# david-cortes/cmfrec

Measured on AMD Instinct MI355X. Metric: ALS rows/sec ((users+items)/iteration time), implicit ALS-CG k=50 fp64, higher is better.
Workload: dtype f64

## Files before the change

### cmfrec_amd/csrc/cg_kernels.hpp

```cpp
#pragma once
#include <hip/hip_runtime.h>
#include <stdint.h>
#include <type_traits>

#include "lanes.hpp"

namespace cmfhip {

constexpr int WAVE = 64;
constexpr int TILE = 64;
constexpr int MAX_W = 8;
#ifndef CMF_CG_WAVES_PER_SIMD
#define CMF_CG_WAVES_PER_SIMD 2
#endif
#ifndef CMF_CG_WAVES_PER_SIMD_F32
#define CMF_CG_WAVES_PER_SIMD_F32 3
#endif
#ifndef CMF_CG_WAVES_PER_SIMD_LOW
#define CMF_CG_WAVES_PER_SIMD_LOW 3
#endif
constexpr int CG_NTSEL_MAX_S = 7;
template <typename T, int W, int NRES_, int NTSEL = 0> constexpr int cg_waves_per_simd()
{
    if (sizeof(T) == 8 && NTSEL == 1 && W <= 8) return CMF_CG_WAVES_PER_SIMD_LOW;
    if (sizeof(T) == 4 && NTSEL == 1 && W <= 4 && NRES_ == 0) return CMF_CG_WAVES_PER_SIMD_F32 + 1;
    return (sizeof(T) == 4 && W <= 4 && NRES_ == 0) ? CMF_CG_WAVES_PER_SIMD_F32 : CMF_CG_WAVES_PER_SIMD;
}
constexpr int CG_NT_LOW = 6;
#ifndef CMF_CG_NT_F32
#define CMF_CG_NT_F32 1
#endif
#ifndef CMF_CG_NT_MIN_S
#define CMF_CG_NT_MIN_S 4
#endif

struct RowDesc {
    int row;
    int nnz;
    unsigned long long st;
};

constexpr int CG_NCOUNTERS = 64;
constexpr int CG_COUNTER_STRIDE = 32;

template <typename T>
__device__ __forceinline__ T cg_div(T num, T den)
{
#ifndef CMF_CG_IEEE_DIV
    if constexpr (sizeof(T) == 4) return num * __builtin_amdgcn_rcpf(den);
    else {
        double y = __builtin_amdgcn_rcp(den);
        double e = __builtin_fma(-den, y, 1.0);
        y = __builtin_fma(y, e, y);
        e = __builtin_fma(-den, y, 1.0);
        y = __builtin_fma(y, e, y);
        double q = num * y;
        const double r = __builtin_fma(-den, q, num);
        return __builtin_fma(r, y, q);
    }
#else
    return num / den;
#endif
}

template <typename V>
__device__ __forceinline__ V lds_g(const V *p) { return *p; }

template <typename T>
struct CgParams {
    T *A;
    size_t lda;
    const T *B;
    size_t ldb;
    int k;
    const size_t *indptr;
    const int *indices;
    const T *values;
    const T *bias_sub;
    const T *weights = nullptr;
    const T *wsum = nullptr;
    const int *order;
    const RowDesc *desc;
    int nrows;
    const T *BtB;
    T lam, lam_last;
    int scale_lam, scale_bias_const;
    int max_cg_steps;
    int precond;
    int koff = 0, kc = 0;
    const T *CtC = nullptr;
    const T *UC = nullptr;
    T w_side = 0;
    int rows_with_u = 0;
    int row_first = 0;
    const size_t *indptr2 = nullptr;
    const int *indices2 = nullptr;
    const T *values2 = nullptr;
    const T *C2 = nullptr;
    int *counter = nullptr;
    int p_side = 0, scale_lam_sideinfo = 0;
    const T *Bi = nullptr;
    const T *BiTBi = nullptr;
    int ki = 0;
    T w_imp = 0;
    const T *rconst = nullptr;
    size_t ldr = 0;
    int gx = 0;
#ifdef CMF_CG_DEBUG
    int dbg = 0;
#endif
#ifdef CMF_CG_TICKS
    unsigned long long *ticks = nullptr;
#endif
};
#ifdef CMF_CG_TICKS
#define CMF_TICK() __builtin_amdgcn_s_memtime()
__device__ __forceinline__ void cg_ticks_flush(unsigned long long *t, int slot, unsigned long long wait, unsigned long long pass, unsigned long long rows,
                                               unsigned long long total, int lane)
{
    if (t != nullptr && lane == 0) {
        atomicAdd(t + 4 * slot + 0, wait); atomicAdd(t + 4 * slot + 1, pass); atomicAdd(t + 4 * slot + 2, rows); atomicAdd(t + 4 * slot + 3, total);
    }
}
#endif
#ifdef CMF_CG_DEBUG
#define CMF_DBG(P, bit) (((P).dbg & (bit)) != 0)
#else
#define CMF_DBG(P, bit) false
#endif
template <int NT, int S, typename TILE, typename T>
__device__ __forceinline__ void dbg_fill_tile(TILE &tile, T val)
{
#pragma unroll
    for (int t = 0; t < NT; t++)
#pragma unroll
        for (int s = 0; s < S; s++) tile.set(t, s, val);
}

template <typename T>
__device__ __forceinline__ T wave_sum(T v) { return lanes::wave_sum(v); }

template <typename T, int NT, int I>
__device__ __forceinline__ T treduce8_low_first(const T (&v)[8], bool h)
{
    if constexpr (I + 4 < NT) {
        T keep = h ? v[I + 4] : v[I];
        return keep + lanes::recv_xor4(v[I], v[I + 4]);
    } else return v[I] + lanes::xor4_lower(v[I]);
}
template <typename T, int NT = 8>
__device__ __forceinline__ T treduce8_low(const T (&v)[8], int lane)
{
    static_assert(NT >= 4 && NT <= 8, "entries per lane group");
    T u[4], q[2];
    bool h = (lane & 4) != 0;
    u[0] = treduce8_low_first<T, NT, 0>(v, h); u[1] = treduce8_low_first<T, NT, 1>(v, h);
    u[2] = treduce8_low_first<T, NT, 2>(v, h); u[3] = treduce8_low_first<T, NT, 3>(v, h);
    h = (lane & 2) != 0;
#pragma unroll
    for (int i = 0; i < 2; i++) {
        T keep = h ? u[i + 2] : u[i];
        T send = h ? u[i] : u[i + 2];
        q[i] = keep + lanes::xor2(send);
    }
    h = (lane & 1) != 0;
    T keep = h ? q[1] : q[0];
    T send = h ? q[0] : q[1];
    return keep + lanes::xor1(send);
}

template <typename T>
__device__ __forceinline__ T treduce8_high(const T (&v)[8], int lane)
{
    T u[4], q[2];
#pragma unroll
    for (int i = 0; i < 4; i++) u[i] = lanes::tswap32_add(v[i], v[i + 4]);
#pragma unroll
    for (int i = 0; i < 2; i++) q[i] = lanes::tswap16_add(u[i], u[i + 2]);
    const bool h = (lane & 8) != 0;
    T keep = h ? q[1] : q[0];
    return keep + lanes::recv_xor8(q[0], q[1]);
}

#ifndef CMF_PASS_VECTOR_LDS
#define CMF_PASS_VECTOR_LDS 2
#endif
template <typename T> constexpr bool pass_vector_in_lds() { return CMF_PASS_VECTOR_LDS == 1 || (CMF_PASS_VECTOR_LDS == 2 && sizeof(T) == 8); }
template <typename T, int S>
__device__ __forceinline__ void replicate(T vdist, T (&vrep)[S], int lane);
template <typename T, int S, int GR = 8>
__device__ __forceinline__ void pass_vector_lds(T vdist, T (&vrep)[S], T (&wts)[8], int lane, T *__restrict__ pv)
{
    const int jj = lane >> 3, ll = lane & 7;
    pv[lane] = vdist;
    __builtin_amdgcn_wave_barrier();
#pragma unroll
    for (int s = 0; s < S; s++) vrep[s] = pv[ll + 8 * s];
    const T *wp = pv + GR * jj;
#pragma unroll
    for (int t = 0; t < GR; t++) wts[t] = wp[t];
    __builtin_amdgcn_wave_barrier();
}

__host__ __device__ constexpr int gram_ld(int S) { return 8 * S + 1; }
#ifndef CMF_GRAM_ROWS_BY_K
#define CMF_GRAM_ROWS_BY_K 1
#endif
template <typename T> __host__ __device__ constexpr int gram_rows(int S) { return (CMF_GRAM_ROWS_BY_K && pass_vector_in_lds<T>()) ? S : 8; }
__host__ __device__ constexpr int gram_ld_rows(int S, int GR)
{
    if (GR == 8) return gram_ld(S);
    int ld = 8 * S;
    while ((S * ld) % 32 != 8 && (S * ld) % 32 != 24) ld++;
    return ld;
}
__host__ __device__ constexpr int gram_ld2(int S) { return 8 * S + 2; }
template <typename T> __host__ __device__ constexpr int gram_elems(int S) { return sizeof(T) == 4 ? 64 * gram_ld2(S) : 64 * gram_ld(S); }
template <typename T, int S, int GR = 8> __device__ __forceinline__ int gram_index(int r, int c)
{
    if constexpr (sizeof(T) == 4) return 2 * ((r >> 1) * gram_ld2(S) + c) + (r & 1);
    else return r * gram_ld_rows(S, GR) + c;
}
template <typename T, int S, int GR = 8>
__device__ __forceinline__ void stage_gramian(T *__restrict__ G, const T *__restrict__ BtB, int k, int tid, int nthreads)
{
    static_assert(GR == 8 || sizeof(T) == 8, "rows by k: double precision");
    for (int e = tid; e < 8 * GR * 8 * S; e += nthreads) {
        const int r = e / (8 * S), c = e % (8 * S);
        G[gram_index<T, S, GR>(r, c)] = (r < k && c < k) ? BtB[(size_t)r * k + c] : T(0);
    }
}

template <typename T, int S>
struct RegTile {
    T v[8][S];
    __device__ __forceinline__ void set(int t, int s, T x) { v[t][s] = x; }
};
typedef float f32x2 __attribute__((ext_vector_type(2)));
template <int S>
struct RegTile<float, S> {
    f32x2 v[4][S];
    __device__ __forceinline__ void set(int t, int s, float x) { v[t >> 1][s][t & 1] = x; }
};

template <typename T>
struct PassAcc {
    T v[8];
    __device__ __forceinline__ void zero()
    {
#pragma unroll
        for (int s = 0; s < 8; s++) v[s] = T(0);
    }
    __device__ __forceinline__ void close(T (&out)[8]) const
    {
#pragma unroll
        for (int s = 0; s < 8; s++) out[s] = v[s];
    }
};
template <>
struct PassAcc<float> {
    f32x2 v[8];
    __device__ __forceinline__ void zero()
    {
#pragma unroll
        for (int s = 0; s < 8; s++) v[s] = f32x2{0.f, 0.f};
    }
    __device__ __forceinline__ void close(float (&out)[8]) const
    {
#pragma unroll
        for (int s = 0; s < 8; s++) out[s] = v[s][0] + v[s][1];
    }
};

#ifndef CMF_CG_EARLY_GATHER
#define CMF_CG_EARLY_GATHER 0
#endif
struct NoAfter {
    template <typename TAG> __device__ __forceinline__ void operator()(TAG) const {}
};
template <int S, typename ACC>
__device__ __forceinline__ void pin_acc(ACC &out)
{
#pragma unroll
    for (int s = 0; s < S; s++) asm volatile("" : "+v"(out.v[s]));
}
template <int TS, typename T, int S, typename TILE>
__device__ __forceinline__ void load_tile_slot(TILE &tile, const char *base, unsigned ldb_bytes, unsigned it, int col_last)
{
    const T *rp = reinterpret_cast<const T *>(base + (unsigned long long)it * ldb_bytes);
#pragma unroll
    for (int s = 0; s < S; s++) tile.set(TS, s, rp[(s < S - 1) ? 8 * s : col_last]);
}

template <typename T, int S, int NT = 8>
__device__ __forceinline__ void load_tile(RegTile<T, S> &tile, const T *__restrict__ Bm, size_t ldb,
                                          int k, int my_idx, int cnt, int lane)
{
    const int jj = lane >> 3, ll = lane & 7;
    int its[8];
    its[0] = lanes::bcast8<0>(my_idx); its[1] = lanes::bcast8<1>(my_idx); its[2] = lanes::bcast8<2>(my_idx);
    its[3] = lanes::bcast8<3>(my_idx);
    if (NT > 4) its[4] = lanes::bcast8<4>(my_idx);
    if (NT > 5) its[5] = lanes::bcast8<5>(my_idx);
    if (NT > 6) its[6] = lanes::bcast8<6>(my_idx);
    if (NT > 7) its[7] = lanes::bcast8<7>(my_idx);
    const int first_idx = __builtin_amdgcn_readfirstlane(my_idx);
    const int col_last = min(ll + 8 * (S - 1), k - 1) - ll;
    const char *base = reinterpret_cast<const char *>(Bm + ll);
    const unsigned ldb_bytes = (unsigned)(ldb * sizeof(T));
#pragma unroll
    for (int t = 0; t < NT; t++) {
        const unsigned it = (unsigned)(((jj * NT + t) < cnt) ? its[t] : first_idx);
        const T *rp = reinterpret_cast<const T *>(base + (unsigned long long)it * ldb_bytes);
#pragma unroll
        for (int s = 0; s < S; s++) tile.set(t, s, rp[(s < S - 1) ? 8 * s : col_last]);
    }
}

template <typename T, bool IMPLICIT, int MODE>
__device__ __forceinline__ T pass_weight(T coef, T x, bool valid, T g = T(1))
{
    T w;
    if (IMPLICIT) {
        if (MODE == 0) w = -(coef - T(1)) * x - coef;
        else           w = coef * (x - T(1)) + coef;
    } else {
        if (MODE == 0) w = -((coef - x) * g);
        else           w = coef * g;
    }
    return valid ? w : T(0);
}

template <typename T>
__device__ __forceinline__ T row_lam_mult(const CgParams<T> &P, int row, int nnz)
{
    return (P.wsum != nullptr) ? P.wsum[row] : (T)nnz;
}
template <typename T, bool IMPLICIT>
__device__ __forceinline__ T entry_weight(const CgParams<T> &P, size_t pos)
{
    if (IMPLICIT) return T(1);
    return (P.weights != nullptr) ? P.weights[pos] : T(1);
}

template <int S, bool IMPLICIT, int MODE, int NT = 8, bool INIT = false, typename AFTER = NoAfter>
__device__ __forceinline__ void tile_pass_f32(const RegTile<float, S> &tile, const float (&vrep)[S], float x, bool valid,
                                          PassAcc<float> &out, int lane, float g = 1.f, AFTER after = AFTER())
{
    static_assert(NT % 2 == 0, "single precision: the entries of a lane group travel in pairs");
    float c[8];
#pragma unroll
    for (int q = 0; q < NT / 2; q++) {
        f32x2 acc = f32x2{0.f, 0.f};
#pragma unroll
        for (int s = 0; s < S; s++) acc += tile.v[q][s] * f32x2{vrep[s], vrep[s]};
        c[2 * q] = acc[0]; c[2 * q + 1] = acc[1];
    }
    float coef = treduce8_low<float, NT>(c, lane);
    const float w = pass_weight<float, IMPLICIT, MODE>(coef, x, valid, g);
    float wts[8];
    wts[0] = lanes::bcast8<0>(w); wts[1] = lanes::bcast8<1>(w); wts[2] = lanes::bcast8<2>(w); wts[3] = lanes::bcast8<3>(w);
    if (NT > 4) { wts[4] = lanes::bcast8<4>(w); wts[5] = lanes::bcast8<5>(w); }
    if (NT > 6) { wts[6] = lanes::bcast8<6>(w); wts[7] = lanes::bcast8<7>(w); }
    if constexpr (std::is_same<AFTER, NoAfter>::value) {
#pragma unroll
    for (int q = 0; q < NT / 2; q++) {
        const f32x2 w2 = f32x2{wts[2 * q], wts[2 * q + 1]};
#pragma unroll
        for (int s = 0; s < S; s++) out.v[s] = (INIT && q == 0) ? w2 * tile.v[q][s] : out.v[s] + w2 * tile.v[q][s];
    }
    } else {
        static_for<0, NT / 2>([&](auto qc) {
            constexpr int q = decltype(qc)::value;
            const f32x2 w2 = f32x2{wts[2 * q], wts[2 * q + 1]};
#pragma unroll
            for (int s = 0; s < S; s++) out.v[s] = (INIT && q == 0) ? w2 * tile.v[q][s] : out.v[s] + w2 * tile.v[q][s];
            pin_acc<S>(out);
            after(std::integral_constant<int, 2 * q>{});
            after(std::integral_constant<int, 2 * q + 1>{});
        });
    }
    if constexpr (INIT) {
#pragma unroll
        for (int s = S; s < 8; s++) out.v[s] = f32x2{0.f, 0.f};
    }
}

template <typename T, int S, bool IMPLICIT, int MODE, int NT = 8, bool INIT = false, typename AFTER = NoAfter>
__device__ __forceinline__ void tile_pass(const RegTile<T, S> &tile, const T (&vrep)[S], T x, bool valid,
                                          PassAcc<T> &out, int lane, T g = T(1), AFTER after = AFTER())
{
    if constexpr (std::is_same<T, float>::value) {
        tile_pass_f32<S, IMPLICIT, MODE, NT, INIT, AFTER>(tile, vrep, x, valid, out, lane, g, after);
    } else {
    T c[8];
#pragma unroll
    for (int t = 0; t < NT; t++) {
        T acc = T(0);
#pragma unroll
        for (int s = 0; s < S; s++) acc += tile.v[t][s] * vrep[s];
        c[t] = acc;
    }
    T coef = treduce8_low<T, NT>(c, lane);
    const T w = pass_weight<T, IMPLICIT, MODE>(coef, x, valid, g);
    T wts[8];
    wts[0] = lanes::bcast8<0>(w); wts[1] = lanes::bcast8<1>(w); wts[2] = lanes::bcast8<2>(w); wts[3] = lanes::bcast8<3>(w);
    if (NT > 4) wts[4] = lanes::bcast8<4>(w);
    if (NT > 5) wts[5] = lanes::bcast8<5>(w);
    if (NT > 6) wts[6] = lanes::bcast8<6>(w);
    if (NT > 7) wts[7] = lanes::bcast8<7>(w);
    if constexpr (std::is_same<AFTER, NoAfter>::value) {
#pragma unroll
    for (int t = 0; t < NT; t++) {
#pragma unroll
        for (int s = 0; s < S; s++) out.v[s] = (INIT && t == 0) ? wts[t] * tile.v[t][s] : out.v[s] + wts[t] * tile.v[t][s];
    }
    } else {
        static_for<0, NT>([&](auto tc) {
            constexpr int t = decltype(tc)::value;
#pragma unroll
            for (int s = 0; s < S; s++) out.v[s] = (INIT && t == 0) ? wts[t] * tile.v[t][s] : out.v[s] + wts[t] * tile.v[t][s];
            pin_acc<S>(out);
            after(tc);
        });
    }
    if constexpr (INIT) {
#pragma unroll
        for (int s = S; s < 8; s++) out.v[s] = T(0);
    }
    }
}

template <typename T, int S, int W>
__device__ __forceinline__ void gram_pass(const T *__restrict__ G, T wdist, PassAcc<T> &out, int lane, int wr)
{
    constexpr int LD = gram_ld(S);
    const int jj = lane >> 3, ll = lane & 7;
    T wts[8];
    wts[0] = lanes::bcast8<0>(wdist); wts[1] = lanes::bcast8<1>(wdist); wts[2] = lanes::bcast8<2>(wdist);
    wts[3] = lanes::bcast8<3>(wdist); wts[4] = lanes::bcast8<4>(wdist); wts[5] = lanes::bcast8<5>(wdist);
    wts[6] = lanes::bcast8<6>(wdist); wts[7] = lanes::bcast8<7>(wdist);
    if constexpr (std::is_same<T, float>::value && W <= 4) {
#pragma unroll
        for (int q = 0; q < 4; q++) {
            if (W > 1 && (q % W) != wr) continue;
            const f32x2 *g = reinterpret_cast<const f32x2 *>(G) + (jj * 4 + q) * gram_ld2(S) + ll;
            const f32x2 w2 = f32x2{wts[2 * q], wts[2 * q + 1]};
#pragma unroll
            for (int s = 0; s < S; s++) out.v[s] += w2 * lds_g(g + 8 * s);
        }
    } else {
#pragma unroll
        for (int t = 0; t < 8; t++) {
            if (W > 1 && (t % W) != wr) continue;
#pragma unroll
            for (int s = 0; s < S; s++) {
                if constexpr (std::is_same<T, float>::value) out.v[s][0] += wts[t] * G[gram_index<T, S>(jj * 8 + t, ll + 8 * s)];
                else out.v[s] += wts[t] * lds_g(G + (jj * 8 + t) * LD + ll + 8 * s);
            }
        }
    }
}

template <bool NEG, typename T, int S, int W, int GR = 8>
__device__ __forceinline__ void gram_pass_w(const T *__restrict__ G, const T (&wts)[8], PassAcc<T> &out, int lane, int wr)
{
    constexpr int LD = gram_ld_rows(S, GR);
    const int jj = lane >> 3, ll = lane & 7;
    if constexpr (std::is_same<T, float>::value && W <= 4) {
#pragma unroll
        for (int q = 0; q < 4; q++) {
            if (W > 1 && (q % W) != wr) continue;
            const f32x2 *g = reinterpret_cast<const f32x2 *>(G) + (jj * 4 + q) * gram_ld2(S) + ll;
            const f32x2 w2 = f32x2{wts[2 * q], wts[2 * q + 1]};
#pragma unroll
            for (int s = 0; s < S; s++) out.v[s] = NEG ? out.v[s] - w2 * lds_g(g + 8 * s) : out.v[s] + w2 * lds_g(g + 8 * s);
        }
    } else {
#pragma unroll
        for (int t = 0; t < GR; t++) {
            if (W > 1 && (t % W) != wr) continue;
#pragma unroll
            for (int s = 0; s < S; s++) {
                if constexpr (std::is_same<T, float>::value) {
                    const float g = G[gram_index<T, S>(jj * 8 + t, ll + 8 * s)];
                    out.v[s][0] = NEG ? out.v[s][0] - wts[t] * g : out.v[s][0] + wts[t] * g;
                } else {
                    const T g = lds_g(G + (jj * GR + t) * LD + ll + 8 * s);
                    out.v[s] = NEG ? out.v[s] - wts[t] * g : out.v[s] + wts[t] * g;
                }
            }
        }
    }
}

template <typename T, int S>
__device__ __forceinline__ void replicate(T vdist, T (&vrep)[S], int lane)
{
    const int ll = lane & 7;
#pragma unroll
    for (int s = 0; s < S; s++) vrep[s] = __shfl(vdist, s * 8 + ll);
}

template <typename T, int S, bool IMPLICIT, int W, int RPB, bool GRAMX = false, int NRES_ = 0, int NTSEL = 0>
__global__ void __launch_bounds__(64 * W * RPB, (cg_waves_per_simd<T, W, NRES_, NTSEL>()))
cg_rows_kernel(const CgParams<T> P)
{
    constexpr bool GRAM = IMPLICIT || GRAMX;
    extern __shared__ __attribute__((aligned(16))) unsigned char smem_raw[];
    T *G = reinterpret_cast<T *>(smem_raw);
    T *red = G + (GRAM ? gram_elems<T>(S) : 0);
    const int tid = threadIdx.x;
    const int lane = tid & 63;
    const int wave = tid >> 6;
    const int grp = wave / W;
    const int wr = wave % W;
    const int k = P.k;

    const int nteams = gridDim.x * RPB;
    __shared__ int s_claim[4];
    constexpr bool PV = pass_vector_in_lds<T>();
    __shared__ __attribute__((aligned(16))) T s_pv[PV ? W * RPB : 1][PV ? 64 : 1];
    const int cslot = (blockIdx.x * RPB + grp) % CG_NCOUNTERS;
    int *const my_counter = P.counter + cslot * CG_COUNTER_STRIDE;
    const int cbase = nteams + cslot;
    auto issue_claim = [&]() -> int {
        int v = 0;
        if (wr == 0 && lane == 0) v = atomicAdd(my_counter, 1);
        return v;
    };
    int rnxt, rnn;
    if (W == 1) {
        const int c1 = issue_claim(), c2 = issue_claim();
        rnxt = cbase + CG_NCOUNTERS * __builtin_amdgcn_readfirstlane(c1);
        rnn = cbase + CG_NCOUNTERS * __builtin_amdgcn_readfirstlane(c2);
    } else if (wr == 0 && lane == 0) {
        s_claim[2] = cbase + CG_NCOUNTERS * atomicAdd(my_counter, 1);
        s_claim[3] = cbase + CG_NCOUNTERS * atomicAdd(my_counter, 1);
    }
    constexpr int GR = gram_rows<T>(S);
    if (GRAM) stage_gramian<T, S, GR>(G, P.BtB, k, tid, blockDim.x);
    if (GRAM || W > 1) __syncthreads();
    if (W > 1) { rnxt = s_claim[2]; rnn = s_claim[3]; }
    T *myred = red + (size_t)grp * 2 * W * 64;

    int buf = 0;
    static_assert(W == 1 || RPB == 1, "multi-wave teams own their workgroup (barriers are per row)");

    constexpr int NRES = NRES_ > 0 ? NRES_ : ((std::is_same<T, float>::value && W == 8) ? 2 : 1);
    static_assert(NRES == 1 || std::is_same<T, float>::value, "two resident tiles: single precision");
    static_assert(NTSEL == 0 || (S >= CMF_CG_NT_MIN_S && (sizeof(T) == 4 || S <= CG_NTSEL_MAX_S) && NRES_ == 0),
                  "launches by tile size: tiles by row length (double precision: k <= 56)");
    constexpr int NT_MIN = (S >= CMF_CG_NT_MIN_S && (CMF_CG_NT_F32 || !std::is_same<T, float>::value)) ? (std::is_same<T, float>::value ? 6 : 5) : 8;
    auto nt_of = [&](int nnz_) -> int {
        int nt = (nnz_ + 8 * W * NRES - 1) / (8 * W * NRES);
        if (std::is_same<T, float>::value) nt = (nt + 1) & ~1;
        return (nt > 8) ? 8 : (nt < NT_MIN ? NT_MIN : nt);
    };
    struct Pre { int idx; T x; T a; int idx2; T x2; T g; T g2; };
    auto load_desc = [&](int rix_) -> RowDesc {
        RowDesc d; d.row = 0; d.nnz = 0; d.st = 0;
        if (rix_ < P.nrows) d = P.desc[rix_];
        d.row = __builtin_amdgcn_readfirstlane(d.row);
        d.nnz = __builtin_amdgcn_readfirstlane(d.nnz);
        d.st = ((unsigned long long)(unsigned)__builtin_amdgcn_readfirstlane((int)(d.st >> 32)) << 32) |
               (unsigned)__builtin_amdgcn_readfirstlane((int)(d.st & 0xffffffffu));
        return d;
    };
    auto load_pre = [&](const RowDesc &d) -> Pre {
        Pre q; q.idx = 0; q.x = T(0); q.a = T(0); q.idx2 = 0; q.x2 = T(0); q.g = T(1); q.g2 = T(1);
        const int nt = nt_of(d.nnz), tl = 8 * nt;
        const int b = lane & 7;
        const int ent = (lane >> 3) * nt + b;
        const int cnt = min(tl, d.nnz - wr * tl);
        if (b < nt && ent < cnt) {
            const size_t pos = d.st + (size_t)wr * tl + ent;
            q.idx = P.indices[pos];
            q.x = P.values[pos];
            q.g = entry_weight<T, IMPLICIT>(P, pos);
            if (!IMPLICIT && P.bias_sub != nullptr) q.x -= P.bias_sub[q.idx];
        }
        if (NRES == 2) {
            const int cnt2 = min(tl, d.nnz - (wr + W) * tl);
            if (b < nt && ent < cnt2) {
                const size_t pos = d.st + (size_t)(wr + W) * tl + ent;
                q.idx2 = P.indices[pos];
                q.x2 = P.values[pos];
                q.g2 = entry_weight<T, IMPLICIT>(P, pos);
                if (!IMPLICIT && P.bias_sub != nullptr) q.x2 -= P.bias_sub[q.idx2];
            }
        }
        if (d.nnz > 0 && lane < k) q.a = P.A[(size_t)d.row * P.lda + lane];
        return q;
    };
    int rix = blockIdx.x * RPB + grp;
    RowDesc dcur = load_desc(rix);
    RowDesc dnxt = load_desc(rnxt);
    Pre pcur = load_pre(dcur);
    int pend = issue_claim();
    constexpr bool EARLY = CMF_CG_EARLY_GATHER != 0;
    constexpr int NT_MAX = (NTSEL == 1) ? CG_NT_LOW : 8;
    RegTile<T, S> tile_c;
    RegTile<T, (NRES == 2) ? S : 1> tile2_c;
    const char *const gbase = reinterpret_cast<const char *>(P.B + (lane & 7));
    const unsigned gldb = (unsigned)(P.ldb * sizeof(T));
    const int gcol_last = min((lane & 7) + 8 * (S - 1), k - 1) - (lane & 7);
    auto gather_slot = [&](auto &tl_, auto tc, int idx_, int first_idx_, int nt_, int cnt_) {
        constexpr int t = decltype(tc)::value;
        if constexpr (t < NT_MAX) {
            if (t < nt_) {
                const unsigned it_ = (unsigned)((((lane >> 3) * nt_ + t) < cnt_) ? lanes::bcast8<t>(idx_) : first_idx_);
                load_tile_slot<t, T, S>(tl_, gbase, gldb, it_, gcol_last);
            }
        }
    };
    struct Want { int nt0, cnt0, nt1, cnt1; };
    auto want_of = [&](const RowDesc &d) -> Want {
        Want w_;
        const int nt = nt_of(d.nnz), tl = 8 * nt;
        w_.cnt0 = min(tl, d.nnz - wr * tl);
        w_.nt0 = (w_.cnt0 > 0 && !CMF_DBG(P, 1)) ? nt : 0;
        w_.cnt1 = (NRES == 2) ? min(tl, d.nnz - (wr + W) * tl) : 0;
        w_.nt1 = (w_.cnt1 > 0 && !CMF_DBG(P, 1)) ? nt : 0;
        return w_;
    };
    auto gather_row = [&](const RowDesc &d, const Pre &q) {
        const Want w_ = want_of(d);
        const int f0 = __builtin_amdgcn_readfirstlane(q.idx);
        static_for<0, NT_MAX>([&](auto tc) { gather_slot(tile_c, tc, q.idx, f0, w_.nt0, w_.cnt0); });
        if constexpr (NRES == 2) {
            const int f1 = __builtin_amdgcn_readfirstlane(q.idx2);
            static_for<0, NT_MAX>([&](auto tc) { gather_slot(tile2_c, tc, q.idx2, f1, w_.nt1, w_.cnt1); });
        }
    };
    if constexpr (EARLY) gather_row(dcur, pcur);
#ifdef CMF_CG_TICKS
    unsigned long long tk_wait = 0, tk_pass = 0, tk_rows = 0;
    const unsigned long long tk_begin = CMF_TICK();
#endif
    int it = 0;
    RowDesc dnn;
    Pre pnxt;
    auto solve_row = [&](auto nt_tag) {
        constexpr int NT = decltype(nt_tag)::value;
        constexpr int TL = 8 * NT;
        const int row = dcur.row;
        const size_t st = dcur.st;
        const int nnz = dcur.nnz;
        const int ntiles = (nnz + TL - 1) / TL;
        const int my_ntiles = (ntiles > wr) ? (ntiles - wr + W - 1) / W : 0;
        const bool resident = NT < 8 || my_ntiles <= NRES;

        T lam = P.lam, lam_last = P.lam_last;
        if (GRAMX && P.kc > 0) {
            if (P.scale_lam || P.scale_lam_sideinfo) {
                T mult = row_lam_mult(P, row, nnz);
                if (P.scale_lam_sideinfo) mult += (T)P.p_side;
                lam *= mult; lam_last *= mult;
            }
        } else if (!IMPLICIT && P.scale_lam) {
            const T mult = row_lam_mult(P, row, nnz);
            lam *= mult;
            if (!P.scale_bias_const) lam_last *= mult;
        }
        T *arow = P.A + (size_t)row * P.lda;
        T a_d = pcur.a;

        RegTile<T, S> tile_r;
        RegTile<T, (NRES == 2) ? S : 1> tile2_r;
        auto &tile = [&]() -> RegTile<T, S> & { if constexpr (EARLY) return tile_c; else return tile_r; }();
        auto &tile2 = [&]() -> RegTile<T, (NRES == 2) ? S : 1> & { if constexpr (EARLY) return tile2_c; else return tile2_r; }();
        const int ent = (lane >> 3) * NT + (lane & 7);
        const bool lane_has = (NT == 8) || (lane & 7) < NT;
        const int cnt0 = min(TL, nnz - wr * TL);
        T x_res = pcur.x;
        const T g_res = pcur.g;
        bool valid_res = lane_has && ent < cnt0;
        if (CMF_DBG(P, 1)) dbg_fill_tile<8, S>(tile, (T)(pcur.idx & 3) * (T)0.001);
        else if (!EARLY && cnt0 > 0) load_tile<T, S, NT>(tile, P.B, P.ldb, k, pcur.idx, cnt0, lane);
        const int cnt1 = (NRES == 2) ? min(TL, nnz - (wr + W) * TL) : 0;
        const T x2_res = pcur.x2, g2_res = pcur.g2;
        const bool valid2_res = lane_has && ent < cnt1;
        if constexpr (NRES == 2) {
            if (!EARLY && cnt1 > 0 && !CMF_DBG(P, 1)) load_tile<T, S, NT>(tile2, P.B, P.ldb, k, pcur.idx2, cnt1, lane);
        }
        dnn = load_desc(rnn);
        pnxt = load_pre(dnxt);
#ifdef CMF_CG_TICKS
        const unsigned long long tk0 = CMF_TICK();
        asm volatile("s_waitcnt vmcnt(0)" ::: "memory");
        const unsigned long long tk1 = CMF_TICK();
        tk_wait += tk1 - tk0;
#endif

        auto run_pass = [&](T vdist, auto mode_tag, bool first, auto fin_tag) -> T {
            constexpr int MODE = decltype(mode_tag)::value;
            constexpr bool FIN = decltype(fin_tag)::value && EARLY;
            asm volatile("" ::: "memory");
            T vrep[S];
            T gw[8];
            if constexpr (PV) pass_vector_lds<T, S, GR>(vdist, vrep, gw, lane, &s_pv[wave][0]);
            else replicate<T, S>(vdist, vrep, lane);
            PassAcc<T> acc;
            acc.zero();
            if constexpr (FIN) {
                if (NT < 8 || NRES == 2 || resident) {
                    const Want nx = want_of(dnxt);
                    const int f0 = __builtin_amdgcn_readfirstlane(pnxt.idx);
                    auto after0 = [&](auto tc) { gather_slot(tile, tc, pnxt.idx, f0, nx.nt0, nx.cnt0); };
                    if (cnt0 > 0 && !CMF_DBG(P, 4)) {
                        tile_pass<T, S, IMPLICIT, MODE, NT>(tile, vrep, x_res, valid_res, acc, lane, g_res, after0);
                        static_for<NT, NT_MAX>(after0);
                    } else static_for<0, NT_MAX>(after0);
                    if constexpr (NRES == 2) {
                        const int f1 = __builtin_amdgcn_readfirstlane(pnxt.idx2);
                        auto after1 = [&](auto tc) { gather_slot(tile2, tc, pnxt.idx2, f1, nx.nt1, nx.cnt1); };
                        if (cnt1 > 0 && !CMF_DBG(P, 4)) {
                            tile_pass<T, S, IMPLICIT, MODE, NT>(tile2, vrep, x2_res, valid2_res, acc, lane, g2_res, after1);
                            static_for<NT, NT_MAX>(after1);
                        } else static_for<0, NT_MAX>(after1);
                    }
                } else {
                for (int tl = wr; tl < ntiles; tl += W) {
                    const int cnt = min(TL, nnz - tl * TL);
                    const bool valid = lane_has && ent < cnt;
                    const size_t pos = st + (size_t)tl * TL + ent;
                    int my_idx = valid ? P.indices[pos] : 0;
                    T x = valid ? P.values[pos] : T(0);
                    const T g = valid ? entry_weight<T, IMPLICIT>(P, pos) : T(1);
                    if (!IMPLICIT && P.bias_sub != nullptr && valid) x -= P.bias_sub[my_idx];
                    if (!CMF_DBG(P, 1)) load_tile<T, S, NT>(tile, P.B, P.ldb, k, my_idx, cnt, lane);
                    if (!CMF_DBG(P, 4)) tile_pass<T, S, IMPLICIT, MODE, NT>(tile, vrep, x, valid, acc, lane, g);
                }
                gather_row(dnxt, pnxt);
                }
            } else
            if constexpr (NRES == 2) {
                if (cnt0 > 0 && !CMF_DBG(P, 4)) tile_pass<T, S, IMPLICIT, MODE, NT>(tile, vrep, x_res, valid_res, acc, lane, g_res);
                if (cnt1 > 0 && !CMF_DBG(P, 4)) tile_pass<T, S, IMPLICIT, MODE, NT>(tile2, vrep, x2_res, valid2_res, acc, lane, g2_res);
            } else if constexpr (NT < 8) {
                if (cnt0 > 0 && !CMF_DBG(P, 4)) tile_pass<T, S, IMPLICIT, MODE, NT>(tile, vrep, x_res, valid_res, acc, lane, g_res);
            } else
            for (int tl = wr; tl < ntiles; tl += W) {
                T x, g; bool valid;
                const bool have = (tl == wr) && (resident || first);
                if (!have) {
                    const int cnt = min(TL, nnz - tl * TL);
                    valid = lane_has && ent < cnt;
                    const size_t pos = st + (size_t)tl * TL + ent;
                    int my_idx = valid ? P.indices[pos] : 0;
                    x = valid ? P.values[pos] : T(0);
                    g = valid ? entry_weight<T, IMPLICIT>(P, pos) : T(1);
                    if (!IMPLICIT && P.bias_sub != nullptr && valid) x -= P.bias_sub[my_idx];
                    if (!CMF_DBG(P, 1)) load_tile<T, S, NT>(tile, P.B, P.ldb, k, my_idx, cnt, lane);
                } else {
                    x = x_res; g = g_res; valid = valid_res;
                }
                if (!CMF_DBG(P, 4)) tile_pass<T, S, IMPLICIT, MODE, NT>(tile, vrep, x, valid, acc, lane, g);
            }
            if (GRAM && !CMF_DBG(P, 2)) {
                if constexpr (PV) gram_pass_w<MODE == 0, T, S, W, GR>(G, gw, acc, lane, wr);
                else gram_pass<T, S, W>(G, (MODE == 0) ? -vdist : vdist, acc, lane, wr);
            }
            T out[8];
            acc.close(out);
            T tot = treduce8_high<T>(out, lane);
            if (W > 1) {
                T *rb = myred + (size_t)buf * W * 64;
                rb[wr * 64 + lane] = tot;
                if (first && wr == 0 && lane == 0) s_claim[it & 1] = cbase + CG_NCOUNTERS * pend;
                __syncthreads();
                tot = T(0);
#pragma unroll
                for (int w = 0; w < W; w++) tot += rb[w * 64 + lane];
                buf ^= 1;
            }
            return tot;
        };

        T r_d = run_pass(a_d, std::integral_constant<int, 0>{}, true, std::false_type{});
        r_d -= lam * a_d;
        if (!IMPLICIT && lam != lam_last && lane == k - 1) r_d -= (lam_last - lam) * a_d;
        if (GRAMX && P.rconst != nullptr && lane < k) r_d += P.rconst[(size_t)row * P.ldr + lane];
        if (lane >= k) r_d = T(0);
        T p_d = r_d;
        T r_old = CMF_DBG(P, 8) ? T(1) : wave_sum(r_d * r_d);
        bool done = (r_old <= (T)1e-12);
        for (int step = 0; step < P.max_cg_steps - (EARLY ? 1 : 0) && !done; step++) {
            T Ap_d = run_pass(p_d, std::integral_constant<int, 1>{}, false, std::false_type{});
            Ap_d += lam * p_d;
            if (!IMPLICIT && lam != lam_last && lane == k - 1) Ap_d += (lam_last - lam) * p_d;
            if (lane >= k) Ap_d = T(0);
            T alpha = CMF_DBG(P, 8) ? T(0.001) : cg_div(r_old, wave_sum(Ap_d * p_d));
            a_d += alpha * p_d;
            if (!EARLY && step == P.max_cg_steps - 1) break;
            r_d -= alpha * Ap_d;
            T r_new = CMF_DBG(P, 8) ? T(0.5) : wave_sum(r_d * r_d);
            if (r_new <= (T)1e-8) done = true;
            else {
                p_d = p_d * cg_div(r_new, r_old) + r_d;
                r_old = r_new;
            }
        }
        if (EARLY && P.max_cg_steps > 0 && !done) {
            T Ap_d = run_pass(p_d, std::integral_constant<int, 1>{}, false, std::true_type{});
            Ap_d += lam * p_d;
            if (!IMPLICIT && lam != lam_last && lane == k - 1) Ap_d += (lam_last - lam) * p_d;
            if (lane >= k) Ap_d = T(0);
            const T alpha = CMF_DBG(P, 8) ? T(0.001) : cg_div(r_old, wave_sum(Ap_d * p_d));
            a_d += alpha * p_d;
        } else if constexpr (EARLY) gather_row(dnxt, pnxt);
#ifdef CMF_CG_TICKS
        tk_pass += CMF_TICK() - tk1; tk_rows += (wr == 0);
#endif
        if (wr == 0 && lane < k) arow[lane] = a_d;
    };
    for (; rix < P.nrows; it++) {
        const int nt = nt_of(dcur.nnz);
        if constexpr (NT_MIN == 8) solve_row(std::integral_constant<int, 8>{});
        else if constexpr (std::is_same<T, float>::value) {
            if constexpr (NTSEL == 1) solve_row(std::integral_constant<int, 6>{});
            else if constexpr (NTSEL == 2) solve_row(std::integral_constant<int, 8>{});
            else if (nt == 6) solve_row(std::integral_constant<int, 6>{});
            else solve_row(std::integral_constant<int, 8>{});
        } else if constexpr (NTSEL == 1) {
            if (nt <= 5) solve_row(std::integral_constant<int, 5>{});
            else solve_row(std::integral_constant<int, 6>{});
        } else if constexpr (NTSEL == 2) {
            if (nt <= 7) solve_row(std::integral_constant<int, 7>{});
            else solve_row(std::integral_constant<int, 8>{});
        } else {
            switch (nt) {
                case 5: solve_row(std::integral_constant<int, 5>{}); break;
                case 6: solve_row(std::integral_constant<int, 6>{}); break;
                case 7: solve_row(std::integral_constant<int, 7>{}); break;
                default: solve_row(std::integral_constant<int, 8>{}); break;
            }
        }
        const int r3 = (W == 1) ? cbase + CG_NCOUNTERS * __builtin_amdgcn_readfirstlane(pend) : s_claim[it & 1];
        dcur = dnxt; dnxt = dnn; pcur = pnxt;
        rix = rnxt; rnxt = rnn; rnn = r3;
        pend = issue_claim();
    }
#ifdef CMF_CG_TICKS
    cg_ticks_flush(P.ticks, W == 1 ? 0 : W == 2 ? 1 : W == 4 ? 2 : 3, tk_wait, tk_pass, tk_rows, CMF_TICK() - tk_begin, lane);
#endif
}

constexpr int TILE4 = 32;

template <typename T, int S>
struct RegTile4 {
    T v[4][S];
    __device__ __forceinline__ void set(int t, int s, T x) { v[t][s] = x; }
    __device__ __forceinline__ T get(int t, int s) const { return v[t][s]; }
};
template <int S>
struct RegTile4<float, S> {
    f32x2 v[2][S];
    __device__ __forceinline__ void set(int t, int s, float x) { v[t >> 1][s][t & 1] = x; }
    __device__ __forceinline__ f32x2 pair0(int s) const { return v[0][s]; }
};

template <typename T, int S>
__device__ __forceinline__ void load_tile4(RegTile4<T, S> &tile, const T *__restrict__ Bm, size_t ldb,
                                           int k, int my_idx, int cnt, int lane)
{
    const int jj = lane >> 3, ll = lane & 7;
    int its[4];
    its[0] = lanes::bcast8<0>(my_idx); its[1] = lanes::bcast8<2>(my_idx);
    its[2] = lanes::bcast8<4>(my_idx); its[3] = lanes::bcast8<6>(my_idx);
    const int first_idx = __builtin_amdgcn_readfirstlane(my_idx);
    const int col_last = min(ll + 8 * (S - 1), k - 1) - ll;
    const char *base = reinterpret_cast<const char *>(Bm + ll);
    const unsigned ldb_bytes = (unsigned)(ldb * sizeof(T));
#pragma unroll
    for (int t = 0; t < 4; t++) {
        const unsigned it = (unsigned)(((jj * 4 + t) < cnt) ? its[t] : first_idx);
        const T *rp = reinterpret_cast<const T *>(base + (unsigned long long)it * ldb_bytes);
#pragma unroll
        for (int s = 0; s < S; s++) tile.set(t, s, rp[(s < S - 1) ? 8 * s : col_last]);
    }
}

template <typename T>
__device__ __forceinline__ T treduce4_low(const T (&v)[4], int lane)
{
    T u[2];
    bool h = (lane & 4) != 0;
#pragma unroll
    for (int i = 0; i < 2; i++) {
        T keep = h ? v[i + 2] : v[i];
        u[i] = keep + lanes::recv_xor4(v[i], v[i + 2]);
    }
    h = (lane & 2) != 0;
    T keep = h ? u[1] : u[0];
    T send = h ? u[0] : u[1];
    T q = keep + lanes::xor2(send);
    return q + lanes::xor1(q);
}

template <int S, bool IMPLICIT, int MODE, typename TILE, bool INIT = false, typename AFTER = NoAfter>
__device__ __forceinline__ void tile_pass4_f32(const TILE &tile, const float (&vrep)[S], float x, bool valid,
                                           PassAcc<float> &out, int lane, float g = 1.f, AFTER after = AFTER())
{
    float c[4];
#pragma unroll
    for (int q = 0; q < 2; q++) {
        f32x2 acc = f32x2{0.f, 0.f};
#pragma unroll
        for (int s = 0; s < S; s++) acc += tile.v[q][s] * f32x2{vrep[s], vrep[s]};
        c[2 * q] = acc[0]; c[2 * q + 1] = acc[1];
    }
    float coef = treduce4_low<float>(c, lane);
    const float w = pass_weight<float, IMPLICIT, MODE>(coef, x, valid, g);
    float wts[4];
    wts[0] = lanes::bcast8<0>(w); wts[1] = lanes::bcast8<2>(w); wts[2] = lanes::bcast8<4>(w); wts[3] = lanes::bcast8<6>(w);
    if constexpr (std::is_same<AFTER, NoAfter>::value) {
#pragma unroll
    for (int q = 0; q < 2; q++) {
        const f32x2 w2 = f32x2{wts[2 * q], wts[2 * q + 1]};
#pragma unroll
        for (int s = 0; s < S; s++) out.v[s] = (INIT && q == 0) ? w2 * tile.v[q][s] : out.v[s] + w2 * tile.v[q][s];
    }
    } else {
        static_for<0, 2>([&](auto qc) {
            constexpr int q = decltype(qc)::value;
            const f32x2 w2 = f32x2{wts[2 * q], wts[2 * q + 1]};
#pragma unroll
            for (int s = 0; s < S; s++) out.v[s] = (INIT && q == 0) ? w2 * tile.v[q][s] : out.v[s] + w2 * tile.v[q][s];
            pin_acc<S>(out);
            after(std::integral_constant<int, 2 * q>{});
            after(std::integral_constant<int, 2 * q + 1>{});
        });
    }
    if constexpr (INIT) {
#pragma unroll
        for (int s = S; s < 8; s++) out.v[s] = f32x2{0.f, 0.f};
    }
}

template <typename T, int S, bool IMPLICIT, int MODE, typename TILE, bool INIT = false, typename AFTER = NoAfter>
__device__ __forceinline__ void tile_pass4(const TILE &tile, const T (&vrep)[S], T x, bool valid,
                                           PassAcc<T> &out, int lane, T g = T(1), AFTER after = AFTER())
{
    if constexpr (std::is_same<T, float>::value) {
        tile_pass4_f32<S, IMPLICIT, MODE, TILE, INIT, AFTER>(tile, vrep, x, valid, out, lane, g, after);
    } else {
    T c[4];
#pragma unroll
    for (int t = 0; t < 4; t++) {
        T acc = T(0);
#pragma unroll
        for (int s = 0; s < S; s++) acc += tile.v[t][s] * vrep[s];
        c[t] = acc;
    }
    T coef = treduce4_low<T>(c, lane);
    const T w = pass_weight<T, IMPLICIT, MODE>(coef, x, valid, g);
    T wts[4];
    wts[0] = lanes::bcast8<0>(w); wts[1] = lanes::bcast8<2>(w); wts[2] = lanes::bcast8<4>(w); wts[3] = lanes::bcast8<6>(w);
    if constexpr (std::is_same<AFTER, NoAfter>::value) {
#pragma unroll
    for (int t = 0; t < 4; t++) {
#pragma unroll
        for (int s = 0; s < S; s++) out.v[s] = (INIT && t == 0) ? wts[t] * tile.v[t][s] : out.v[s] + wts[t] * tile.v[t][s];
    }
    } else {
        static_for<0, 4>([&](auto tc) {
            constexpr int t = decltype(tc)::value;
#pragma unroll
            for (int s = 0; s < S; s++) out.v[s] = (INIT && t == 0) ? wts[t] * tile.v[t][s] : out.v[s] + wts[t] * tile.v[t][s];
            pin_acc<S>(out);
            after(tc);
        });
    }
    if constexpr (INIT) {
#pragma unroll
        for (int s = S; s < 8; s++) out.v[s] = T(0);
    }
    }
}

template <typename T, int S>
struct RegTile2 {
    T v[2][S];
    __device__ __forceinline__ void set(int t, int s, T x) { v[t][s] = x; }
    __device__ __forceinline__ T get(int t, int s) const { return v[t][s]; }
};
template <int S>
struct RegTile2<float, S> {
    f32x2 v[S];
    __device__ __forceinline__ void set(int t, int s, float x) { v[s][t] = x; }
    __device__ __forceinline__ f32x2 pair0(int s) const { return v[s]; }
};

template <typename T, int S, typename TILE>
__device__ __forceinline__ void load_tile2(TILE &tile, const T *__restrict__ Bm, size_t ldb,
                                           int k, int my_idx, int cnt, int lane)
{
    const int jj = lane >> 3, ll = lane & 7;
    int its[2];
    its[0] = lanes::bcast8<0>(my_idx); its[1] = lanes::bcast8<4>(my_idx);
    const int first_idx = __builtin_amdgcn_readfirstlane(my_idx);
    const int col_last = min(ll + 8 * (S - 1), k - 1) - ll;
    const char *base = reinterpret_cast<const char *>(Bm + ll);
    const unsigned ldb_bytes = (unsigned)(ldb * sizeof(T));
#pragma unroll
    for (int t = 0; t < 2; t++) {
        const unsigned it = (unsigned)(((jj * 2 + t) < cnt) ? its[t] : first_idx);
        const T *rp = reinterpret_cast<const T *>(base + (unsigned long long)it * ldb_bytes);
#pragma unroll
        for (int s = 0; s < S; s++) tile.set(t, s, rp[(s < S - 1) ? 8 * s : col_last]);
    }
}

template <typename T>
__device__ __forceinline__ T treduce2_low(const T (&v)[2], int lane)
{
    const bool h = (lane & 4) != 0;
    T u = (h ? v[1] : v[0]) + lanes::recv_xor4(v[0], v[1]);
    u += lanes::xor2(u);
    return u + lanes::xor1(u);
}

template <typename T, int S, bool IMPLICIT, int MODE, typename TILE, bool INIT = false, typename AFTER = NoAfter>
__device__ __forceinline__ void tile_pass2(const TILE &tile, const T (&vrep)[S], T x, bool valid,
                                           PassAcc<T> &out, int lane, T g = T(1), AFTER after = AFTER())
{
    T c[2];
    if constexpr (std::is_same<T, float>::value) {
        f32x2 acc = f32x2{0.f, 0.f};
#pragma unroll
        for (int s = 0; s < S; s++) acc += tile.pair0(s) * f32x2{vrep[s], vrep[s]};
        c[0] = acc[0]; c[1] = acc[1];
    } else {
#pragma unroll
        for (int t = 0; t < 2; t++) {
            T acc = T(0);
#pragma unroll
            for (int s = 0; s < S; s++) acc += tile.get(t, s) * vrep[s];
            c[t] = acc;
        }
    }
    const T coef = treduce2_low<T>(c, lane);
    const T w = pass_weight<T, IMPLICIT, MODE>(coef, x, valid, g);
    const T w0 = lanes::bcast8<0>(w), w1 = lanes::bcast8<4>(w);
    if constexpr (std::is_same<T, float>::value) {
        const f32x2 w2 = f32x2{w0, w1};
#pragma unroll
        for (int s = 0; s < S; s++) out.v[s] = INIT ? w2 * tile.pair0(s) : out.v[s] + w2 * tile.pair0(s);
        if constexpr (!std::is_same<AFTER, NoAfter>::value) pin_acc<S>(out);
        after(std::integral_constant<int, 0>{});
        after(std::integral_constant<int, 1>{});
        if constexpr (INIT) {
#pragma unroll
            for (int s = S; s < 8; s++) out.v[s] = f32x2{0.f, 0.f};
        }
    } else {
#pragma unroll
        for (int s = 0; s < S; s++) out.v[s] = INIT ? w0 * tile.get(0, s) : out.v[s] + w0 * tile.get(0, s);
        if constexpr (!std::is_same<AFTER, NoAfter>::value) pin_acc<S>(out);
        after(std::integral_constant<int, 0>{});
#pragma unroll
        for (int s = 0; s < S; s++) out.v[s] += w1 * tile.get(1, s);
        if constexpr (!std::is_same<AFTER, NoAfter>::value) pin_acc<S>(out);
        after(std::integral_constant<int, 1>{});
        if constexpr (INIT) {
#pragma unroll
            for (int s = S; s < 8; s++) out.v[s] = T(0);
        }
    }
}

template <typename T, int S, int NE> struct TinyTile { using type = RegTile4<T, S>; };
template <typename T, int S> struct TinyTile<T, S, 2> { using type = RegTile2<T, S>; };

#ifndef CMF_TINY_WAVES_PER_SIMD
#define CMF_TINY_WAVES_PER_SIMD 4
#endif
#ifndef CMF_TINY_GREG_F32
#define CMF_TINY_GREG_F32 1
#endif
#ifndef CMF_TINY_GREG_F64
#define CMF_TINY_GREG_F64 1
#endif
template <typename T, bool GRAM> constexpr bool tiny_greg() { return GRAM && (sizeof(T) == 8 ? CMF_TINY_GREG_F64 != 0 : CMF_TINY_GREG_F32 != 0); }
template <typename T, bool GRAM> constexpr int tiny_waves_per_simd() { return tiny_greg<T, GRAM>() ? (sizeof(T) == 8 ? 2 : 3) : CMF_TINY_WAVES_PER_SIMD; }
template <typename T, int S, int GR = 8>
struct GramRegs {
    T v[GR][S];
    __device__ __forceinline__ void load(const T *__restrict__ G, int lane)
    {
        const int jj = lane >> 3, ll = lane & 7;
#pragma unroll
        for (int t = 0; t < GR; t++)
#pragma unroll
            for (int s = 0; s < S; s++) v[t][s] = G[gram_index<T, S, GR>(jj * GR + t, ll + 8 * s)];
    }
};
template <int S>
struct GramRegs<float, S, 8> {
    f32x2 v[4][S];
    __device__ __forceinline__ void load(const float *__restrict__ G, int lane)
    {
        const int jj = lane >> 3, ll = lane & 7;
#pragma unroll
        for (int q = 0; q < 4; q++) {
            const f32x2 *g = reinterpret_cast<const f32x2 *>(G) + (jj * 4 + q) * gram_ld2(S) + ll;
#pragma unroll
            for (int s = 0; s < S; s++) v[q][s] = g[8 * s];
        }
    }
};
template <int S>
// ... 746 lines not shown
```

Measured before the change: 170.2 million.

## Run CG scalar updates on a leader wave and broadcast direction via LDS

```diff
diff --git a/cmfrec_amd/csrc/cg_kernels.hpp b/cmfrec_amd/csrc/cg_kernels.hpp
--- a/cmfrec_amd/csrc/cg_kernels.hpp
+++ b/cmfrec_amd/csrc/cg_kernels.hpp
@@ -202,6 +202,18 @@
     __builtin_amdgcn_wave_barrier();
 }
 
+template <typename T, int S, int GR = 8>
+__device__ __forceinline__ void pass_vector_read(T (&vrep)[S], T (&wts)[8], int lane, const T *pv)
+{
+    const int jj = lane >> 3, ll = lane & 7;
+#pragma unroll
+    for (int s = 0; s < S; s++) vrep[s] = pv[ll + 8 * s];
+    const T *wp = pv + GR * jj;
+#pragma unroll
+    for (int t = 0; t < GR; t++) wts[t] = wp[t];
+    __builtin_amdgcn_wave_barrier();
+}
+
 __host__ __device__ constexpr int gram_ld(int S) { return 8 * S + 1; }
 #ifndef CMF_GRAM_ROWS_BY_K
 #define CMF_GRAM_ROWS_BY_K 1
@@ -275,6 +287,17 @@
 #ifndef CMF_CG_EARLY_GATHER
 #define CMF_CG_EARLY_GATHER 0
 #endif
+#ifndef CMF_CG_TEAM_LEADER
+#define CMF_CG_TEAM_LEADER 1
+#endif
+#ifndef CMF_CG_TEAM_LEADER_W
+#define CMF_CG_TEAM_LEADER_W (4 | 8)
+#endif
+template <typename T, int W, int S = 0, bool GRAMX = false, int NTSEL = 0> constexpr bool cg_team_leader()
+{
+    constexpr bool SPILLS = GRAMX && W == 8 && S == 7 && NTSEL == 1;
+    return CMF_CG_TEAM_LEADER != 0 && CMF_CG_EARLY_GATHER == 0 && W > 1 && pass_vector_in_lds<T>() && ((CMF_CG_TEAM_LEADER_W) & W) != 0 && !SPILLS;
+}
 struct NoAfter {
     template <typename TAG> __device__ __forceinline__ void operator()(TAG) const {}
 };
@@ -520,7 +543,10 @@
     const int nteams = gridDim.x * RPB;
     __shared__ int s_claim[4];
     constexpr bool PV = pass_vector_in_lds<T>();
-    __shared__ __attribute__((aligned(16))) T s_pv[PV ? W * RPB : 1][PV ? 64 : 1];
+    constexpr bool LEAD = cg_team_leader<T, W, S, GRAMX, NTSEL>();
+    __shared__ __attribute__((aligned(16))) T s_pv[PV ? (LEAD ? 1 : W * RPB) : 1][PV ? 64 : 1];
+    __shared__ int s_done;
+    const bool lead = __builtin_amdgcn_readfirstlane(wr) == 0;
     const int cslot = (blockIdx.x * RPB + grp) % CG_NCOUNTERS;
     int *const my_counter = P.counter + cslot * CG_COUNTER_STRIDE;
     const int cbase = nteams + cslot;
@@ -699,6 +725,11 @@
             asm volatile("" ::: "memory");
             T vrep[S];
             T gw[8];
+            if constexpr (LEAD) {
+                if (first) s_pv[0][lane] = vdist;
+                __builtin_amdgcn_wave_barrier();
+                pass_vector_read<T, S, GR>(vrep, gw, lane, &s_pv[0][0]);
+            } else
             if constexpr (PV) pass_vector_lds<T, S, GR>(vdist, vrep, gw, lane, &s_pv[wave][0]);
             else replicate<T, S>(vdist, vrep, lane);
             PassAcc<T> acc;
@@ -770,14 +801,61 @@
                 rb[wr * 64 + lane] = tot;
                 if (first && wr == 0 && lane == 0) s_claim[it & 1] = cbase + CG_NCOUNTERS * pend;
                 __syncthreads();
-                tot = T(0);
-#pragma unroll
-                for (int w = 0; w < W; w++) tot += rb[w * 64 + lane];
+                if (!LEAD || lead) {
+                    tot = T(0);
+#pragma unroll
+                    for (int w = 0; w < W; w++) tot += rb[w * 64 + lane];
+                }
                 buf ^= 1;
             }
             return tot;
         };
 
+        if constexpr (LEAD) {
+            const int nsteps = P.max_cg_steps;
+            T r_d = run_pass(a_d, std::integral_constant<int, 0>{}, true, std::false_type{});
+            if (nsteps > 0) {
+                T p_d = T(0), r_old = T(0);
+                if (lead) {
+                    r_d -= lam * a_d;
+                    if (!IMPLICIT && lam != lam_last && lane == k - 1) r_d -= (lam_last - lam) * a_d;
+                    if (GRAMX && P.rconst != nullptr && lane < k) r_d += P.rconst[(size_t)row * P.ldr + lane];
+                    if (lane >= k) r_d = T(0);
+                    p_d = r_d;
+                    r_old = CMF_DBG(P, 8) ? T(1) : wave_sum(r_d * r_d);
+                    s_pv[0][lane] = p_d;
+                    if (lane == 0) s_done = (r_old <= (T)1e-12) ? 1 : 0;
+                }
+                __syncthreads();
+                bool done = __builtin_amdgcn_readfirstlane(s_done) != 0;
+                for (int step = 0; !done; step++) {
+                    T Ap_d = run_pass(p_d, std::integral_constant<int, 1>{}, false, std::false_type{});
+                    const bool last = (step == nsteps - 1);
+                    if (lead) {
+                        Ap_d += lam * p_d;
+                        if (!IMPLICIT && lam != lam_last && lane == k - 1) Ap_d += (lam_last - lam) * p_d;
+                        if (lane >= k) Ap_d = T(0);
+                        T alpha = CMF_DBG(P, 8) ? T(0.001) : cg_div(r_old, wave_sum(Ap_d * p_d));
+                        a_d += alpha * p_d;
+                        if (!last) {
+                            r_d -= alpha * Ap_d;
+                            T r_new = CMF_DBG(P, 8) ? T(0.5) : wave_sum(r_d * r_d);
+                            int dn = 1;
+                            if (!(r_new <= (T)1e-8)) {
+                                p_d = p_d * cg_div(r_new, r_old) + r_d;
+                                r_old = r_new;
+                                dn = 0;
+                            }
+                            s_pv[0][lane] = p_d;
+                            if (lane == 0) s_done = dn;
+                        }
+                    }
+                    if (last) break;
+                    __syncthreads();
+                    done = __builtin_amdgcn_readfirstlane(s_done) != 0;
+                }
+            }
+        } else {
         T r_d = run_pass(a_d, std::integral_constant<int, 0>{}, true, std::false_type{});
         r_d -= lam * a_d;
         if (!IMPLICIT && lam != lam_last && lane == k - 1) r_d -= (lam_last - lam) * a_d;
@@ -810,6 +888,7 @@
             const T alpha = CMF_DBG(P, 8) ? T(0.001) : cg_div(r_old, wave_sum(Ap_d * p_d));
             a_d += alpha * p_d;
         } else if constexpr (EARLY) gather_row(dnxt, pnxt);
+        }
 #ifdef CMF_CG_TICKS
         tk_pass += CMF_TICK() - tk1; tk_rows += (wr == 0);
 #endif
```

New measurement: 170.2 million. About the same (-0.0%).
